# PaddlePaddle/Parakeet

Measured on NVIDIA H100. Metric: audio-samples/sec, higher is better.
Workload: dtype bf16x3 (split-bf16 operands, fp32 accumulate; fp32-grade, 1e-3 parity)

## Files before the change

parakeet_b200/csrc/pwg.cu:

```cuda
#include <stdlib.h>
#include <string.h>

#include <algorithm>

#include "pk_host.h"
#include "pk_sm90.cuh"

namespace pk {

constexpr int kPwgR = 64;
constexpr int kPwgG = 128;
constexpr int kPwgS = 64;
constexpr int kPwgStages = 2;
constexpr int kPwgTile = 128 * kSwizzleBytes;
constexpr int kPwgStageBytes = 4 * kPwgTile;
constexpr int kPwgW2Bytes = 2 * kPwgTile;
constexpr int kPwgSmem = kPwgStages * kPwgStageBytes + kPwgW2Bytes + 1024 + 256;
static_assert(kPwgSmem <= 227 * 1024, "shared memory budget");
constexpr int kPwgConsumerThreads = 256;
constexpr int kPwgThreads = kPwgConsumerThreads + 128;
constexpr int kPwgG1Chunks = 5;

struct PwgLayerArgs {
  int batch, t, dil, aux_ch;
  int tiles_per_b, total_tiles;
  const int32_t* lens;
  float gate_c[128];
  float out_b[64];
  float k_a, k_g;
  float* skip;
  int skip_init;
  __nv_bfloat16* y_hi;
  __nv_bfloat16* y_lo;
};

struct PwgTileIter {
  int idx, step, tiles_per_b, total, t;
  const int32_t* lens;
  __device__ PwgTileIter(const PwgLayerArgs& p) : idx(static_cast<int>(blockIdx.x) - static_cast<int>(gridDim.x)),
      step(gridDim.x), tiles_per_b(p.tiles_per_b), total(p.total_tiles), t(p.t), lens(p.lens) {}
  __device__ bool next(int& b, int& m0) {
    for (;;) {
      idx += step;
      if (idx >= total) return false;
      b = idx / tiles_per_b;
      m0 = (idx % tiles_per_b) * 128;
      const int len = lens ? min(__ldg(lens + b), t) : t;
      if (m0 < len) return true;
    }
  }
};

__global__ void __launch_bounds__(kPwgThreads, 1)
pwg_layer_kernel(const __grid_constant__ CUtensorMap tm_x_hi, const __grid_constant__ CUtensorMap tm_x_lo,
                 const __grid_constant__ CUtensorMap tm_c_hi, const __grid_constant__ CUtensorMap tm_c_lo,
                 const __grid_constant__ CUtensorMap tm_w1_hi, const __grid_constant__ CUtensorMap tm_w1_lo,
                 const __grid_constant__ CUtensorMap tm_w2_hi, const __grid_constant__ CUtensorMap tm_w2_lo,
                 const PwgLayerArgs p) {
  extern __shared__ uint8_t smem_raw[];
  const uint32_t smem = (smem_u32(smem_raw) + 1023u) & ~1023u;
  const uint32_t w2 = smem + kPwgStages * kPwgStageBytes;
  const uint32_t bars = w2 + kPwgW2Bytes;
  const uint32_t full_bar = bars;
  const uint32_t empty_bar = full_bar + 8 * kPwgStages;
  const uint32_t w_bar = empty_bar + 8 * kPwgStages;

  const int warp = threadIdx.x >> 5;
  const int lane = threadIdx.x & 31;

  if (threadIdx.x == kPwgConsumerThreads) {
    tma_prefetch_desc(&tm_x_hi); tma_prefetch_desc(&tm_x_lo); tma_prefetch_desc(&tm_c_hi); tma_prefetch_desc(&tm_c_lo);
    tma_prefetch_desc(&tm_w1_hi); tma_prefetch_desc(&tm_w1_lo); tma_prefetch_desc(&tm_w2_hi); tma_prefetch_desc(&tm_w2_lo);
    for (int s = 0; s < kPwgStages; ++s) { mbar_init_a(full_bar + 8 * s, 1); mbar_init_a(empty_bar + 8 * s, kPwgConsumerThreads / 32); }
    mbar_init_a(w_bar, 1);
    fence_barrier_init();
  }
  __syncthreads();

  if (warp >= kPwgConsumerThreads / 32) {
    setmaxnreg_dec<40>();
    if (warp == kPwgConsumerThreads / 32 && lane == 0) {
      mbar_arrive_expect_tx_a(w_bar, kPwgW2Bytes);
      tma_load_3d_a(w2, &tm_w2_hi, w_bar, 0, 0, 0);
      tma_load_3d_a(w2 + kPwgTile, &tm_w2_lo, w_bar, 0, 0, 0);
      uint32_t it = 0;
      PwgTileIter ti(p);
      int b, m0;
      while (ti.next(b, m0)) {
        for (int j = 0; j < kPwgG1Chunks; ++j, ++it) {
          const int s = it % kPwgStages;
          mbar_wait_a(empty_bar + 8 * s, ((it / kPwgStages) & 1) ^ 1);
          const uint32_t st = smem + s * kPwgStageBytes;
          const uint32_t fb = full_bar + 8 * s;
          mbar_arrive_expect_tx_a(fb, kPwgStageBytes);
          const int wj = j == 0 ? 0 : j == 1 ? 2 : j == 2 ? 3 : j == 3 ? 4 : 1;
          if (wj < 3) {
            const int row = m0 + (wj - 1) * p.dil;
            tma_load_3d_a(st, &tm_x_hi, fb, 0, row, b);
            tma_load_3d_a(st + kPwgTile, &tm_x_lo, fb, 0, row, b);
          } else {
            tma_load_3d_a(st, &tm_c_hi, fb, (wj - 3) * kChunkK, m0, b);
            tma_load_3d_a(st + kPwgTile, &tm_c_lo, fb, (wj - 3) * kChunkK, m0, b);
          }
          tma_load_3d_a(st + 2 * kPwgTile, &tm_w1_hi, fb, wj * kChunkK, 0, 0);
          tma_load_3d_a(st + 3 * kPwgTile, &tm_w1_lo, fb, wj * kChunkK, 0, 0);
        }
      }
    }
  } else {
    setmaxnreg_inc<232>();
    const int wg = warp >> 2;
    const int rl = 16 * (warp & 3) + (lane >> 2);
    const int cq = 2 * (lane & 3);
    const int aux_tail_ksteps = ((p.aux_ch - kChunkK) + kWgmmaK - 1) / kWgmmaK;
    const float kSqrtHalf = 0.70710678118654752440f;
    mbar_wait_a(w_bar, 0);
    uint32_t it = 0;
    PwgTileIter ti(p);
    int b, m0;
    while (ti.next(b, m0)) {
      float acc1[64], acc2[64];
      for (int j = 0; j < kPwgG1Chunks; ++j, ++it) {
        const int s = it % kPwgStages;
        mbar_wait_a(full_bar + 8 * s, (it / kPwgStages) & 1);
        const uint32_t st = smem + s * kPwgStageBytes;
        const uint32_t sa = st + wg * 64 * kSwizzleBytes;
        const uint64_t a_hi = make_smem_desc_sw128(sa), a_lo = make_smem_desc_sw128(sa + kPwgTile);
        const uint64_t b_hi = make_smem_desc_sw128(st + 2 * kPwgTile), b_lo = make_smem_desc_sw128(st + 3 * kPwgTile);
        const int ksteps = j == 3 ? aux_tail_ksteps : 4;
        wgmma_fence();
        for (int k = 0; k < ksteps; ++k) {
          wgmma_ss_n128(acc1, a_hi + desc_kstep(k), b_hi + desc_kstep(k), !(j == 0 && k == 0));
          wgmma_ss_n128(acc1, a_lo + desc_kstep(k), b_hi + desc_kstep(k), 1);
          wgmma_ss_n128(acc1, a_hi + desc_kstep(k), b_lo + desc_kstep(k), 1);
        }
        wgmma_commit();
        if (j == kPwgG1Chunks - 1) {
#pragma unroll
          for (int jj = 0; jj < 8; ++jj) {
#pragma unroll
            for (int hh = 0; hh < 2; ++hh) {
              const int r = rl + 8 * hh;
              const uint32_t off = r * kSwizzleBytes + ((((8 * jj + cq) >> 3) ^ (r & 7)) << 4) + (cq & 7) * 2;
              const uint32_t xh = lds_u32(sa + off), xl = lds_u32(sa + kPwgTile + off);
              acc2[4 * jj + 2 * hh] = 0.f;
              acc2[4 * jj + 2 * hh + 1] = 0.f;
              acc2[32 + 4 * jj + 2 * hh] = __uint_as_float(xh << 16) + __uint_as_float(xl << 16);
              acc2[32 + 4 * jj + 2 * hh + 1] = __uint_as_float(xh & 0xffff0000u) + __uint_as_float(xl & 0xffff0000u);
            }
          }
        }
        wgmma_wait<0>();
        reg_fence(acc1);
        __syncwarp();
        if (lane == 0) mbar_arrive_a(empty_bar + 8 * s);
      }
      uint32_t zh[16], zl[16];
#pragma unroll
      for (int jj = 0; jj < 8; ++jj) {
        float z[4];
#pragma unroll
        for (int e = 0; e < 4; ++e) {
          const int c = 8 * jj + cq + (e & 1);
          const float e1 = ex2_approx(fminf(fmaf(acc1[4 * jj + e], p.k_a, p.gate_c[c]), 60.f));
          const float e2 = ex2_approx(fmaf(acc1[32 + 4 * jj + e], p.k_g, p.gate_c[64 + c]));
          const float t1 = 1.f + e1;
          z[e] = (1.f - e1) * rcp_approx(fmaf(t1, e2, t1));
        }
        split2(z[0], z[1], zh[2 * jj], zl[2 * jj]);
        split2(z[2], z[3], zh[2 * jj + 1], zl[2 * jj + 1]);
      }
      const uint64_t b2_hi = make_smem_desc_sw128(w2), b2_lo = make_smem_desc_sw128(w2 + kPwgTile);
      wgmma_fence();
#pragma unroll
      for (int k = 0; k < 4; ++k) {
        const uint32_t ah[4] = {zh[4 * k], zh[4 * k + 1], zh[4 * k + 2], zh[4 * k + 3]};
        const uint32_t al[4] = {zl[4 * k], zl[4 * k + 1], zl[4 * k + 2], zl[4 * k + 3]};
        wgmma_rs_n128(acc2, ah, b2_hi + desc_kstep(k), 1);
        wgmma_rs_n128(acc2, al, b2_hi + desc_kstep(k), 1);
        wgmma_rs_n128(acc2, ah, b2_lo + desc_kstep(k), 1);
      }
      wgmma_commit();
      wgmma_wait<0>();
      reg_fence(acc2);
      const int len = p.lens ? min(__ldg(p.lens + b), p.t) : p.t;
#pragma unroll
      for (int hh = 0; hh < 2; ++hh) {
        const int trow = m0 + wg * 64 + rl + 8 * hh;
        if (trow < p.t) {
          const long long row_off = (static_cast<long long>(b) * p.t + trow) * 64;
          const bool live = trow < len;
#pragma unroll
          for (int jj = 0; jj < 8; ++jj) {
            const int c = 8 * jj + cq;
            float* d2 = p.skip + row_off + c;
            const float s0 = acc2[4 * jj + 2 * hh], s1 = acc2[4 * jj + 2 * hh + 1];
            if (p.skip_init) *reinterpret_cast<float2*>(d2) = make_float2(s0, s1);
            else asm volatile("red.global.add.v2.f32 [%0], {%1, %2};" ::"l"(d2), "f"(s0), "f"(s1) : "memory");
            const float y0 = live ? (acc2[32 + 4 * jj + 2 * hh] + p.out_b[c]) * kSqrtHalf : 0.f;
            const float y1 = live ? (acc2[32 + 4 * jj + 2 * hh + 1] + p.out_b[c + 1]) * kSqrtHalf : 0.f;
            uint32_t oh, ol;
            split2(y0, y1, oh, ol);
            *reinterpret_cast<uint32_t*>(p.y_hi + row_off + c) = oh;
            *reinterpret_cast<uint32_t*>(p.y_lo + row_off + c) = ol;
          }
        }
      }
    }
  }
}

constexpr int kUpMaxStages = 4;
constexpr int kUpMaxScale = 16;
struct UpsampleArgs {
  int n_stages;
  int scale[kUpMaxStages];
  float poly[kUpMaxStages][3][kUpMaxScale];
  int aux, frames, window;
  int hop;
};

__device__ __forceinline__ int floordiv(int a, int b) { return a >= 0 ? a / b : -((-a + b - 1) / b); }

constexpr int kCinFrames = 16;
__global__ void __launch_bounds__(320)
pwg_conv_in_kernel(const float* __restrict__ mel, const float* __restrict__ w_in, int aux, int frames, int window,
                   float* __restrict__ m_out) {
  extern __shared__ float cin_smem[];
  const int kin = 2 * window + 1;
  const int wrow = aux * kin;
  const int pitch = aux + 1;
  float* sw = cin_smem;
  float* sm = sw + wrow * pitch;
  const int span = kCinFrames + kin - 1;
  const int f0 = blockIdx.x * kCinFrames, b = blockIdx.y;
  const int mel_len = frames + 2 * window;
  for (int idx = threadIdx.x; idx < aux * wrow; idx += blockDim.x) {
    const int ch = idx / wrow, r = idx - ch * wrow;
    sw[r * pitch + ch] = __ldg(w_in + idx);
  }
  for (int idx = threadIdx.x; idx < aux * span; idx += blockDim.x) {
    const int ci = idx / span, i = idx - ci * span;
    const int f = f0 + i;
    sm[idx] = f < mel_len ? __ldg(mel + (static_cast<long long>(b) * aux + ci) * mel_len + f) : 0.f;
  }
  __syncthreads();
  const int fg = threadIdx.x / 80, lane_ch = threadIdx.x - fg * 80;
  for (int ch = lane_ch; ch < aux; ch += 80) {
    float acc[4] = {0.f, 0.f, 0.f, 0.f};
    for (int ci = 0; ci < aux; ++ci) {
      const float* mp = sm + ci * span + fg * 4;
      const float* wp = sw + (ci * kin) * pitch + ch;
      for (int q = 0; q < kin; ++q) {
        const float wv = wp[q * pitch];
#pragma unroll
        for (int i = 0; i < 4; ++i) acc[i] = fmaf(wv, mp[q + i], acc[i]);
      }
    }
#pragma unroll
    for (int i = 0; i < 4; ++i) {
      const int f = f0 + fg * 4 + i;
      if (f < frames) m_out[(static_cast<long long>(b) * frames + f) * aux + ch] = acc[i];
    }
  }
}

__global__ void __launch_bounds__(256)
pwg_upsample_kernel(const float* __restrict__ m,
                    const int32_t* __restrict__ frame_lens,
                    const UpsampleArgs a, float* __restrict__ c_f32 ,
                    __nv_bfloat16* __restrict__ c_hi, __nv_bfloat16* __restrict__ c_lo ) {
  extern __shared__ float up_smem[];
  __shared__ float s_poly[kUpMaxStages][3][kUpMaxScale];
  const int j = blockIdx.x, b = blockIdx.y;
  const int aux = a.aux;
  const int n_frames = frame_lens ? min(__ldg(frame_lens + b), a.frames) : a.frames;
  for (int i = threadIdx.x; i < kUpMaxStages * 3 * kUpMaxScale; i += blockDim.x) (&s_poly[0][0][0])[i] = (&a.poly[0][0][0])[i];
  int lo[kUpMaxStages + 1], hi[kUpMaxStages + 1], len[kUpMaxStages + 1];
  len[0] = n_frames;
#pragma unroll
  for (int k = 0; k < kUpMaxStages; ++k) len[k + 1] = k < a.n_stages ? len[k] * a.scale[k] : 0;
#pragma unroll
  for (int k = kUpMaxStages; k >= 0; --k) {
    if (k == a.n_stages) { lo[k] = j * a.hop; hi[k] = (j + 1) * a.hop; }
    else if (k < a.n_stages) {
      const int s = a.scale[k];
      lo[k] = floordiv(lo[k + 1], s) - 1;
      hi[k] = floordiv(hi[k + 1] - 1, s) + 2;
    } else { lo[k] = 0; hi[k] = 0; }
  }
  float* buf[kUpMaxStages + 1];
  int width[kUpMaxStages + 1];
  {
    float* ptr = up_smem;
#pragma unroll
    for (int k = 0; k <= kUpMaxStages; ++k) {
      width[k] = hi[k] - lo[k];
      buf[k] = ptr;
      if (k < a.n_stages) ptr += aux * width[k];
    }
  }
  const int last = a.n_stages - 1;
  for (int idx = threadIdx.x; idx < aux * width[0]; idx += blockDim.x) {
    const int i = idx / aux, ch = idx - i * aux;
    const int f = lo[0] + i;
    const float v = (f >= 0 && f < n_frames) ? __ldg(m + (static_cast<long long>(b) * a.frames + f) * aux + ch) : 0.f;
    buf[0][idx] = v;
  }
  __syncthreads();
#pragma unroll
  for (int k = 0; k + 1 < kUpMaxStages; ++k) {
    if (k + 1 < a.n_stages) {
      const int s = a.scale[k];
      for (int idx = threadIdx.x; idx < aux * width[k + 1]; idx += blockDim.x) {
        const int tt = idx / aux, ch = idx - tt * aux;
        const int t = lo[k + 1] + tt;
        float acc = 0.f;
        if (t >= 0 && t < len[k + 1]) {
          const int mm = t / s, r = t - mm * s;
          const float* in = buf[k] + (mm - 1 - lo[k]) * aux + ch;
          acc = s_poly[k][0][r] * in[0];
          acc = fmaf(s_poly[k][1][r], in[aux], acc);
          acc = fmaf(s_poly[k][2][r], in[2 * aux], acc);
        }
        buf[k + 1][idx] = acc;
      }
      __syncthreads();
    }
  }
  {
    const int k = last;
    const int s = a.scale[k];
    const long long T = static_cast<long long>(a.frames) * a.hop;
    const int groups = aux / 8;
    const float* src = buf[k];
    for (int idx = threadIdx.x; idx < a.hop * groups; idx += blockDim.x) {
      const int tt = idx / groups, g = idx - tt * groups;
      const int t = lo[k + 1] + tt;
      const bool live = t < len[k + 1];
      const int mm = t / s, r = t - mm * s;
      const float p0 = s_poly[k][0][r], p1 = s_poly[k][1][r], p2 = s_poly[k][2][r];
      float v[8];
      if (live) {
        const float4* in = reinterpret_cast<const float4*>(src + (mm - 1 - lo[k]) * aux + g * 8);
        const int pitch4 = aux / 4;
        const float4 a0 = in[0], a1 = in[1], b0 = in[pitch4], b1 = in[pitch4 + 1], c0 = in[2 * pitch4], c1 = in[2 * pitch4 + 1];
        v[0] = fmaf(p2, c0.x, fmaf(p1, b0.x, p0 * a0.x)); v[1] = fmaf(p2, c0.y, fmaf(p1, b0.y, p0 * a0.y));
        v[2] = fmaf(p2, c0.z, fmaf(p1, b0.z, p0 * a0.z)); v[3] = fmaf(p2, c0.w, fmaf(p1, b0.w, p0 * a0.w));
        v[4] = fmaf(p2, c1.x, fmaf(p1, b1.x, p0 * a1.x)); v[5] = fmaf(p2, c1.y, fmaf(p1, b1.y, p0 * a1.y));
        v[6] = fmaf(p2, c1.z, fmaf(p1, b1.z, p0 * a1.z)); v[7] = fmaf(p2, c1.w, fmaf(p1, b1.w, p0 * a1.w));
      } else {
#pragma unroll
        for (int e = 0; e < 8; ++e) v[e] = 0.f;
      }
      if (c_f32) {
#pragma unroll
        for (int e = 0; e < 8; ++e) c_f32[(static_cast<long long>(b) * aux + g * 8 + e) * T + t] = v[e];
      }
      if (c_hi) {
        uint4 h, l;
        split8(v, h, l);
        const long long o = (static_cast<long long>(b) * T + t) * aux + g * 8;
        *reinterpret_cast<uint4*>(c_hi + o) = h;
        *reinterpret_cast<uint4*>(c_lo + o) = l;
      }
    }
  }
}

__global__ void pwg_first_conv_kernel(const float* __restrict__ noise, const float* __restrict__ w, const float* __restrict__ bias,
                                      const int32_t* __restrict__ lens, int t_len, long long total_rows,
                                      __nv_bfloat16* __restrict__ x_hi, __nv_bfloat16* __restrict__ x_lo) {
  const long long n = total_rows * 8;
  for (long long idx = blockIdx.x * static_cast<long long>(blockDim.x) + threadIdx.x; idx < n;
       idx += static_cast<long long>(gridDim.x) * blockDim.x) {
    const long long row = idx >> 3;
    const int g = idx & 7;
    const int b = row / t_len, t = row % t_len;
    const bool live = lens == nullptr || t < __ldg(lens + b);
    const float xv = __ldg(noise + row);
    float v[8];
#pragma unroll
    for (int e = 0; e < 8; ++e) v[e] = live ? fmaf(__ldg(w + g * 8 + e), xv, __ldg(bias + g * 8 + e)) : 0.f;
    uint4 h, l;
    split8(v, h, l);
    reinterpret_cast<uint4*>(x_hi)[idx] = h;
    reinterpret_cast<uint4*>(x_lo)[idx] = l;
  }
}

__global__ void __launch_bounds__(128)
pwg_tail_kernel(const float* __restrict__ skip, const float* __restrict__ skip_bias ,
                const float* __restrict__ w1 , const float* __restrict__ b1,
                const float* __restrict__ w2 , const float* __restrict__ b2, float scale, long long rows,
                float* __restrict__ out) {
  __shared__ float4 sw1[16 * 64];
  __shared__ float sb1[64], sw2[64], ssb[64];
  for (int i = threadIdx.x; i < 64 * 16; i += blockDim.x) {
    const int o = i >> 4, kq = i & 15;
    sw1[kq * 64 + o] = reinterpret_cast<const float4*>(w1)[i];
  }
  if (threadIdx.x < 64) {
    sb1[threadIdx.x] = b1[threadIdx.x];
    sw2[threadIdx.x] = w2[threadIdx.x];
    ssb[threadIdx.x] = skip_bias ? skip_bias[threadIdx.x] : 0.f;
  }
  __syncthreads();
  const float bias2 = __ldg(b2);
  const long long pairs = (rows + 1) >> 1;
  for (long long pr = blockIdx.x * static_cast<long long>(blockDim.x) + threadIdx.x; pr < pairs;
       pr += static_cast<long long>(gridDim.x) * blockDim.x) {
    const long long r0 = pr, r1 = pr + pairs;
    const bool has1 = r1 < rows;
    const float4* p0 = reinterpret_cast<const float4*>(skip + r0 * 64);
    const float4* p1 = reinterpret_cast<const float4*>(skip + (has1 ? r1 : r0) * 64);
    float h0[64], h1[64];
#pragma unroll
    for (int o = 0; o < 64; ++o) { h0[o] = sb1[o]; h1[o] = sb1[o]; }
#pragma unroll 1
    for (int kc = 0; kc < 4; ++kc) {
      float s0[16], s1[16];
#pragma unroll
      for (int q = 0; q < 4; ++q) {
        const float4 u = __ldg(p0 + kc * 4 + q), v = __ldg(p1 + kc * 4 + q);
        const float* sbp = ssb + kc * 16 + q * 4;
        s0[4 * q] = fmaxf((u.x + sbp[0]) * scale, 0.f); s0[4 * q + 1] = fmaxf((u.y + sbp[1]) * scale, 0.f);
        s0[4 * q + 2] = fmaxf((u.z + sbp[2]) * scale, 0.f); s0[4 * q + 3] = fmaxf((u.w + sbp[3]) * scale, 0.f);
        s1[4 * q] = fmaxf((v.x + sbp[0]) * scale, 0.f); s1[4 * q + 1] = fmaxf((v.y + sbp[1]) * scale, 0.f);
        s1[4 * q + 2] = fmaxf((v.z + sbp[2]) * scale, 0.f); s1[4 * q + 3] = fmaxf((v.w + sbp[3]) * scale, 0.f);
      }
#pragma unroll
      for (int q = 0; q < 4; ++q) {
#pragma unroll
        for (int o = 0; o < 64; ++o) {
          const float4 w = sw1[(kc * 4 + q) * 64 + o];
          h0[o] = fmaf(w.x, s0[4 * q], h0[o]); h0[o] = fmaf(w.y, s0[4 * q + 1], h0[o]);
          h0[o] = fmaf(w.z, s0[4 * q + 2], h0[o]); h0[o] = fmaf(w.w, s0[4 * q + 3], h0[o]);
          h1[o] = fmaf(w.x, s1[4 * q], h1[o]); h1[o] = fmaf(w.y, s1[4 * q + 1], h1[o]);
          h1[o] = fmaf(w.z, s1[4 * q + 2], h1[o]); h1[o] = fmaf(w.w, s1[4 * q + 3], h1[o]);
        }
      }
    }
    float y0 = bias2, y1 = bias2;
#pragma unroll
    for (int o = 0; o < 64; ++o) {
      y0 = fmaf(sw2[o], fmaxf(h0[o], 0.f), y0);
      y1 = fmaf(sw2[o], fmaxf(h1[o], 0.f), y1);
    }
    out[r0] = y0;
    if (has1) out[r1] = y1;
  }
}

}

extern "C" int pk_pwg_residual_layer(const pk_pwg_layer_args* a, pk_stream_t stream) {
  PK_CHECK_ARG(a != nullptr, "args is NULL");
  PK_CHECK_ARG(a->batch > 0 && a->t > 0 && a->dilation >= 1, "bad batch/t/dilation");
  PK_CHECK_ARG(a->aux_channels > 64 && a->aux_channels <= 128 && (a->aux_channels % 8) == 0,
               "aux_channels must be in (64,128] and a multiple of 8 (got %d)", a->aux_channels);
  PK_CHECK_ARG(a->x_hi && a->x_lo && a->y_hi && a->y_lo && a->c_hi && a->c_lo && a->w1_hi && a->w1_lo && a->w2_hi && a->w2_lo &&
               a->bias1 && a->bias2 && a->skip, "NULL pointer in pk_pwg_layer_args");
  PK_CHECK_ARG(a->x_hi != a->y_hi, "layer output must not alias its input (neighbouring tiles read the input halo)");
  using namespace pk;
  CUtensorMap tx_hi, tx_lo, tc_hi, tc_lo, tw1_hi, tw1_lo, tw2_hi, tw2_lo;
  int rc;
  const uint64_t T = a->t, B = a->batch;
  const uint32_t w_box_rows = 128;
  if ((rc = encode_tmap_bf16_3d(&tx_hi, a->x_hi, kPwgR, T, B, kPwgR, T * kPwgR, 128))) return rc;
  if ((rc = encode_tmap_bf16_3d(&tx_lo, a->x_lo, kPwgR, T, B, kPwgR, T * kPwgR, 128))) return rc;
  if ((rc = encode_tmap_bf16_3d(&tc_hi, a->c_hi, a->aux_channels, T, B, a->aux_channels, T * a->aux_channels, 128))) return rc;
  if ((rc = encode_tmap_bf16_3d(&tc_lo, a->c_lo, a->aux_channels, T, B, a->aux_channels, T * a->aux_channels, 128))) return rc;
  const uint64_t k1 = kPwgG1Chunks * kChunkK;
  const uint64_t k1_valid = 3 * kChunkK + a->aux_channels;
  if ((rc = encode_tmap_bf16_3d(&tw1_hi, a->w1_hi, k1_valid, kPwgG, 1, k1, k1 * kPwgG, w_box_rows))) return rc;
  if ((rc = encode_tmap_bf16_3d(&tw1_lo, a->w1_lo, k1_valid, kPwgG, 1, k1, k1 * kPwgG, w_box_rows))) return rc;
  if ((rc = encode_tmap_bf16_3d(&tw2_hi, a->w2_hi, 64, 128, 1, 64, 0, w_box_rows))) return rc;
  if ((rc = encode_tmap_bf16_3d(&tw2_lo, a->w2_lo, 64, 128, 1, 64, 0, w_box_rows))) return rc;
  int resident = 0;
  if ((rc = prepare_kernel(pwg_layer_kernel, kPwgThreads, kPwgSmem, &resident))) return rc;
  PwgLayerArgs p;
  p.batch = a->batch; p.t = a->t; p.dil = a->dilation; p.aux_ch = a->aux_channels;
  p.tiles_per_b = (a->t + 127) / 128;
  p.total_tiles = p.tiles_per_b * a->batch;
  p.lens = a->lens; p.skip = a->skip; p.skip_init = a->skip_init;
  p.k_a = kGateKa; p.k_g = kGateKg;
  fold_gate_bias(p.gate_c, a->bias1, 64);
  for (int i = 0; i < 64; ++i) p.out_b[i] = a->bias2[64 + i];
  p.y_hi = static_cast<__nv_bfloat16*>(a->y_hi); p.y_lo = static_cast<__nv_bfloat16*>(a->y_lo);
  const cudaStream_t st = static_cast<cudaStream_t>(stream);
  const int grid = std::min(p.total_tiles, resident);
  pwg_layer_kernel<<<grid, kPwgThreads, kPwgSmem, st>>>(tx_hi, tx_lo, tc_hi, tc_lo, tw1_hi, tw1_lo, tw2_hi, tw2_lo, p);
  PK_CHECK_CUDA(cudaGetLastError());
  count_launch();
  return PK_OK;
}

extern "C" int pk_pwg_upsample(const float* mel, const float* conv_in_w, const float* fir, const int32_t* scales,
                               int32_t n_stages, int32_t batch, int32_t aux, int32_t frames, int32_t window,
                               const int32_t* frame_lens, float* conv_in_ws, float* c_f32, void* c_hi, void* c_lo,
                               pk_stream_t stream) {
  using namespace pk;
  PK_CHECK_ARG(mel && conv_in_w && fir && scales && conv_in_ws, "NULL pointer");
  PK_CHECK_ARG(n_stages >= 1 && n_stages <= kUpMaxStages, "n_stages must be in [1,%d]", kUpMaxStages);
  PK_CHECK_ARG(batch > 0 && aux > 0 && frames > 0 && window >= 0, "bad sizes");
  PK_CHECK_ARG((c_hi == nullptr) == (c_lo == nullptr), "c_hi and c_lo must both be set or both NULL");
  PK_CHECK_ARG((aux % 8) == 0, "aux must be a multiple of 8 (got %d)", aux);
  UpsampleArgs a;
  memset(&a, 0, sizeof(a));
  a.n_stages = n_stages; a.aux = aux; a.frames = frames; a.window = window; a.hop = 1;
  for (int k = 0; k < n_stages; ++k) {
    const int s = scales[k];
    PK_CHECK_ARG(s >= 1 && s <= kUpMaxScale, "upsample scale %d unsupported (max %d)", s, kUpMaxScale);
    a.scale[k] = s;
    a.hop *= s;
    for (int r = 0; r < s; ++r)
      for (int q = 0; q < 2 * s + 1; ++q) a.poly[k][(r + q) / s][r] += fir[q];
    fir += 2 * s + 1;
  }
  const cudaStream_t st = static_cast<cudaStream_t>(stream);
  {
    const int kin = 2 * window + 1;
    const size_t cin_smem = (static_cast<size_t>(aux) * kin * (aux + 1) + static_cast<size_t>(aux) * (kCinFrames + kin - 1)) * sizeof(float);
    PK_CHECK_ARG(cin_smem <= 220 * 1024, "conv_in weight does not fit shared memory (%zu bytes)", cin_smem);
    if (int rc = prepare_kernel(pwg_conv_in_kernel, 320, cin_smem)) return rc;
    dim3 cgrid((frames + kCinFrames - 1) / kCinFrames, batch);
    pwg_conv_in_kernel<<<cgrid, 320, cin_smem, st>>>(mel, conv_in_w, aux, frames, window, conv_in_ws);
    PK_CHECK_CUDA(cudaGetLastError());
    count_launch();
  }
  if (c_f32 == nullptr && c_hi == nullptr) return PK_OK;
  size_t floats = 0;
  {
    int w = a.hop;
    for (int k = n_stages - 1; k >= 0; --k) {
      w = (w - 1) / a.scale[k] + 4;
      floats += static_cast<size_t>(aux) * w;
    }
  }
  const size_t smem = floats * sizeof(float);
  PK_CHECK_ARG(smem <= 200 * 1024, "upsample tile does not fit shared memory (%zu bytes)", smem);
  if (int rc = prepare_kernel(pwg_upsample_kernel, 256, smem)) return rc;
  dim3 grid(frames, batch);
  pwg_upsample_kernel<<<grid, 256, smem, st>>>(conv_in_ws, frame_lens, a, c_f32, static_cast<__nv_bfloat16*>(c_hi),
                                               static_cast<__nv_bfloat16*>(c_lo));
  PK_CHECK_CUDA(cudaGetLastError());
  count_launch();
  return PK_OK;
}

extern "C" int pk_pwg_first_conv(const float* noise, const float* w, const float* bias, const int32_t* lens, int32_t batch,
                                 int32_t t, void* x_hi, void* x_lo, pk_stream_t stream) {
  PK_CHECK_ARG(noise && w && bias && x_hi && x_lo, "NULL pointer");
  PK_CHECK_ARG(batch > 0 && t > 0, "bad sizes");
  const long long rows = static_cast<long long>(batch) * t;
  const int threads = 256;
  const int blocks = static_cast<int>(std::min<long long>((rows * 8 + threads - 1) / threads, pk::sm_count() * 16LL));
  pk::pwg_first_conv_kernel<<<blocks, threads, 0, static_cast<cudaStream_t>(stream)>>>(
      noise, w, bias, lens, t, rows, static_cast<__nv_bfloat16*>(x_hi), static_cast<__nv_bfloat16*>(x_lo));
  PK_CHECK_CUDA(cudaGetLastError());
  pk::count_launch();
  return PK_OK;
}

extern "C" int pk_pwg_tail(const float* skip, const float* skip_bias, const float* w1, const float* b1, const float* w2,
                           const float* b2, float scale, int64_t rows, float* out, pk_stream_t stream) {
  PK_CHECK_ARG(skip && w1 && b1 && w2 && b2 && out, "NULL pointer");
  PK_CHECK_ARG(rows > 0, "bad sizes");
  const int threads = 128;
  const long long pairs = (rows + 1) / 2;
  const int blocks = static_cast<int>(std::min<long long>((pairs + threads - 1) / threads, pk::sm_count() * 12LL));
  pk::pwg_tail_kernel<<<blocks, threads, 0, static_cast<cudaStream_t>(stream)>>>(skip, skip_bias, w1, b1, w2, b2, scale, rows, out);
  PK_CHECK_CUDA(cudaGetLastError());
  pk::count_launch();
  return PK_OK;
}
```

Measured before the change: 72.29 million.

## Split tail-kernel output channels across lane pairs to cut per-thread registers

The tail kernel now has each pair of adjacent lanes share one row pair, with each lane computing half of the 64 hidden outputs. This halves the per-thread accumulator arrays, and __launch_bounds__(128,3) asks for higher occupancy. The shared weight layout is interleaved so the two halves read neighbouring float4 entries, and the second-layer dot product is combined through a shuffle. The trade-off is more passes over skip loads per row (each lane loads the full 64 inputs redundantly), double the grid size, and a serialized shuffle reduction.

```diff
diff --git a/parakeet_b200/csrc/pwg.cu b/parakeet_b200/csrc/pwg.cu
--- a/parakeet_b200/csrc/pwg.cu
+++ b/parakeet_b200/csrc/pwg.cu
@@ -389,7 +389,7 @@
   }
 }
 
-__global__ void __launch_bounds__(128)
+__global__ void __launch_bounds__(128, 3)
 pwg_tail_kernel(const float* __restrict__ skip, const float* __restrict__ skip_bias ,
                 const float* __restrict__ w1 , const float* __restrict__ b1,
                 const float* __restrict__ w2 , const float* __restrict__ b2, float scale, long long rows,
@@ -398,7 +398,7 @@
   __shared__ float sb1[64], sw2[64], ssb[64];
   for (int i = threadIdx.x; i < 64 * 16; i += blockDim.x) {
     const int o = i >> 4, kq = i & 15;
-    sw1[kq * 64 + o] = reinterpret_cast<const float4*>(w1)[i];
+    sw1[kq * 64 + 2 * (o & 31) + (o >> 5)] = reinterpret_cast<const float4*>(w1)[i];
   }
   if (threadIdx.x < 64) {
     sb1[threadIdx.x] = b1[threadIdx.x];
@@ -407,33 +407,37 @@
   }
   __syncthreads();
   const float bias2 = __ldg(b2);
+  const int lane = threadIdx.x & 31, h = lane & 1;
   const long long pairs = (rows + 1) >> 1;
-  for (long long pr = blockIdx.x * static_cast<long long>(blockDim.x) + threadIdx.x; pr < pairs;
-       pr += static_cast<long long>(gridDim.x) * blockDim.x) {
-    const long long r0 = pr, r1 = pr + pairs;
-    const bool has1 = r1 < rows;
+  const long long warps = static_cast<long long>(gridDim.x) * (blockDim.x >> 5);
+  for (long long pw = (blockIdx.x * static_cast<long long>(blockDim.x >> 5) + (threadIdx.x >> 5)) * 16; pw < pairs; pw += warps * 16) {
+    const long long pr = pw + (lane >> 1);
+    const bool has0 = pr < pairs;
+    const long long r0 = has0 ? pr : pw, r1 = pr + pairs;
+    const bool has1 = has0 && r1 < rows;
     const float4* p0 = reinterpret_cast<const float4*>(skip + r0 * 64);
     const float4* p1 = reinterpret_cast<const float4*>(skip + (has1 ? r1 : r0) * 64);
-    float h0[64], h1[64];
-#pragma unroll
-    for (int o = 0; o < 64; ++o) { h0[o] = sb1[o]; h1[o] = sb1[o]; }
+    float h0[32], h1[32];
+#pragma unroll
+    for (int o = 0; o < 32; ++o) { h0[o] = sb1[32 * h + o]; h1[o] = sb1[32 * h + o]; }
 #pragma unroll 1
-    for (int kc = 0; kc < 4; ++kc) {
-      float s0[16], s1[16];
-#pragma unroll
-      for (int q = 0; q < 4; ++q) {
-        const float4 u = __ldg(p0 + kc * 4 + q), v = __ldg(p1 + kc * 4 + q);
-        const float* sbp = ssb + kc * 16 + q * 4;
+    for (int kc = 0; kc < 8; ++kc) {
+      float s0[8], s1[8];
+#pragma unroll
+      for (int q = 0; q < 2; ++q) {
+        const float4 u = __ldg(p0 + kc * 2 + q), v = __ldg(p1 + kc * 2 + q);
+        const float* sbp = ssb + kc * 8 + q * 4;
         s0[4 * q] = fmaxf((u.x + sbp[0]) * scale, 0.f); s0[4 * q + 1] = fmaxf((u.y + sbp[1]) * scale, 0.f);
         s0[4 * q + 2] = fmaxf((u.z + sbp[2]) * scale, 0.f); s0[4 * q + 3] = fmaxf((u.w + sbp[3]) * scale, 0.f);
         s1[4 * q] = fmaxf((v.x + sbp[0]) * scale, 0.f); s1[4 * q + 1] = fmaxf((v.y + sbp[1]) * scale, 0.f);
         s1[4 * q + 2] = fmaxf((v.z + sbp[2]) * scale, 0.f); s1[4 * q + 3] = fmaxf((v.w + sbp[3]) * scale, 0.f);
       }
 #pragma unroll
-      for (int q = 0; q < 4; ++q) {
-#pragma unroll
-        for (int o = 0; o < 64; ++o) {
-          const float4 w = sw1[(kc * 4 + q) * 64 + o];
+      for (int q = 0; q < 2; ++q) {
+        const float4* wq = sw1 + (kc * 2 + q) * 64 + h;
+#pragma unroll
+        for (int o = 0; o < 32; ++o) {
+          const float4 w = wq[2 * o];
           h0[o] = fmaf(w.x, s0[4 * q], h0[o]); h0[o] = fmaf(w.y, s0[4 * q + 1], h0[o]);
           h0[o] = fmaf(w.z, s0[4 * q + 2], h0[o]); h0[o] = fmaf(w.w, s0[4 * q + 3], h0[o]);
           h1[o] = fmaf(w.x, s1[4 * q], h1[o]); h1[o] = fmaf(w.y, s1[4 * q + 1], h1[o]);
@@ -442,13 +446,24 @@
       }
     }
     float y0 = bias2, y1 = bias2;
-#pragma unroll
-    for (int o = 0; o < 64; ++o) {
-      y0 = fmaf(sw2[o], fmaxf(h0[o], 0.f), y0);
-      y1 = fmaf(sw2[o], fmaxf(h1[o], 0.f), y1);
-    }
-    out[r0] = y0;
-    if (has1) out[r1] = y1;
+    if (h == 0) {
+#pragma unroll
+      for (int o = 0; o < 32; ++o) {
+        y0 = fmaf(sw2[o], fmaxf(h0[o], 0.f), y0);
+        y1 = fmaf(sw2[o], fmaxf(h1[o], 0.f), y1);
+      }
+    }
+    y0 = __shfl_xor_sync(0xffffffffu, y0, 1);
+    y1 = __shfl_xor_sync(0xffffffffu, y1, 1);
+    if (h == 1) {
+#pragma unroll
+      for (int o = 0; o < 32; ++o) {
+        y0 = fmaf(sw2[32 + o], fmaxf(h0[o], 0.f), y0);
+        y1 = fmaf(sw2[32 + o], fmaxf(h1[o], 0.f), y1);
+      }
+      if (has0) out[r0] = y0;
+      if (has1) out[r1] = y1;
+    }
   }
 }
 
@@ -569,7 +584,7 @@
   PK_CHECK_ARG(rows > 0, "bad sizes");
   const int threads = 128;
   const long long pairs = (rows + 1) / 2;
-  const int blocks = static_cast<int>(std::min<long long>((pairs + threads - 1) / threads, pk::sm_count() * 12LL));
+  const int blocks = static_cast<int>(std::min<long long>((pairs + 63) / 64, pk::sm_count() * 12LL));
   pk::pwg_tail_kernel<<<blocks, threads, 0, static_cast<cudaStream_t>(stream)>>>(skip, skip_bias, w1, b1, w2, b2, scale, rows, out);
   PK_CHECK_CUDA(cudaGetLastError());
   pk::count_launch();
```

Result: no change. 72.31 million, median of 6 (+0.0%).
